# nihalsid/single-view-3d-reconstruction

Measured on AMD Instinct MI355X. Metric: query-points/sec fwd+bwd (128^3 grid, 50k pts), higher is better.
Workload: dtype f32

## Files before the change

### single-view-3d-reconstruction_amd/csrc/conv3d_bwdw_bf16.hip

```cpp
#include "common.h"
#include "f16x3.h"

namespace svr {
void colsum_launch(const float *Y, int64_t ldy, float *out, float *part, int64_t M, int64_t N, hipStream_t s);
int64_t colsum_workspace_floats(int64_t M, int64_t N);
void conv3d_bwd_weight_reduce_launch(const float *slab, float *dWp, int Ci, int Co, int cit, int cot, int parts,
                                     hipStream_t s, int param_layout, const float *dbpart, float *db, int dbparts);
}

using namespace svr;

namespace {

typedef __bf16 bf16x8 __attribute__((ext_vector_type(8)));
typedef __bf16 bf16x2 __attribute__((ext_vector_type(2)));
typedef float f32x16 __attribute__((ext_vector_type(16)));

struct ConvShape {
  int B, D, H, W, Ci, Co;
};

constexpr int BRZ = 4, BRY = 4, BRX = 8;
constexpr int HLY = BRY + 2;
constexpr int HROWS = (BRZ + 2) * (BRY + 2);
constexpr int ROWDW = 6;
constexpr int CIS = HROWS * ROWDW + 2;
constexpr int COS = BRZ * BRY * 4 + 4;
constexpr int IN_PLANE = 32 * CIS, DO_PLANE = 32 * COS;
constexpr int BUF = 2 * IN_PLANE + 2 * DO_PLANE;
constexpr int NT = 512;
constexpr int IN_ITEMS = HROWS * 5 * 8;
constexpr int DO_ITEMS = BRZ * BRY * 4 * 8;
constexpr int IN_IT = (IN_ITEMS + NT - 1) / NT;
static_assert(IN_IT == 3 && DO_ITEMS == NT, "prefetch phases below are written for 3 + 1 items per thread");
constexpr int TAPS_PER_WAVE = 7;

__device__ __forceinline__ void split2(float x0, float x1, uint32_t &hi, uint32_t &mid) {
#if defined(SVR_WG_EXP) && SVR_WG_EXP == 3
  hi = __float_as_uint(x0);
  mid = __float_as_uint(x1);
  return;
#endif
  f32x2 v = {x0, x1};
  bf16x2 h = __builtin_convertvector(v, bf16x2);
  hi = __builtin_bit_cast(uint32_t, h);
  f32x2 r = {x0 - __uint_as_float(hi << 16), x1 - __uint_as_float(hi & 0xffff0000u)};
  bf16x2 m = __builtin_convertvector(r, bf16x2);
  mid = __builtin_bit_cast(uint32_t, m);
}

__device__ __forceinline__ bf16x8 frag(uint32_t a, uint32_t b, uint32_t c, uint32_t d) {
  union { uint4 q; bf16x8 v; } f;
  f.q = make_uint4(a, b, c, d);
  return f.v;
}

template <int G, bool F16>
__device__ __forceinline__ void wgrad_rows(const uint32_t *__restrict__ ibuf, const uint32_t *__restrict__ dbuf, int l31, int r,
                                           f32x16 (&acc)[TAPS_PER_WAVE]) {
  constexpr int T0 = G * TAPS_PER_WAVE, T1 = (T0 + TAPS_PER_WAVE < 27) ? T0 + TAPS_PER_WAVE : 27;
  const int vz = r >> 2, vy = r & 3;
  const uint4 bh = *reinterpret_cast<const uint4 *>(dbuf + l31 * COS + r * 4);
  const uint4 bm = *reinterpret_cast<const uint4 *>(dbuf + DO_PLANE + l31 * COS + r * 4);
  const bf16x8 b_hi = frag(bh.x, bh.y, bh.z, bh.w), b_mid = frag(bm.x, bm.y, bm.z, bm.w);
#pragma unroll
  for (int R = T0 / 3; R <= (T1 - 1) / 3; ++R) {
    const int dzi = R / 3, dyi = R % 3;
    const uint32_t *ph = ibuf + l31 * CIS + ((vz + dzi) * HLY + vy + dyi) * ROWDW;
    const uint2 m01 = *reinterpret_cast<const uint2 *>(ph + IN_PLANE), m23 = *reinterpret_cast<const uint2 *>(ph + IN_PLANE + 2);
    const uint32_t m4 = ph[IN_PLANE + 4];
    const uint2 h01 = *reinterpret_cast<const uint2 *>(ph), h23 = *reinterpret_cast<const uint2 *>(ph + 2);
    const uint32_t h4 = ph[4];
#pragma unroll
    for (int dx = 0; dx < 3; ++dx) {
      const int tap = R * 3 + dx;
      if (tap < T0 || tap >= T1) continue;
      const int i = tap - T0;
      const bf16x8 am = dx == 0 ? frag(m01.x, m01.y, m23.x, m23.y)
                      : dx == 2 ? frag(m01.y, m23.x, m23.y, m4)
                                : frag(__builtin_amdgcn_alignbit(m01.y, m01.x, 16), __builtin_amdgcn_alignbit(m23.x, m01.y, 16),
                                       __builtin_amdgcn_alignbit(m23.y, m23.x, 16), __builtin_amdgcn_alignbit(m4, m23.y, 16));
      const bf16x8 ah = dx == 0 ? frag(h01.x, h01.y, h23.x, h23.y)
                      : dx == 2 ? frag(h01.y, h23.x, h23.y, h4)
                                : frag(__builtin_amdgcn_alignbit(h01.y, h01.x, 16), __builtin_amdgcn_alignbit(h23.x, h01.y, 16),
                                       __builtin_amdgcn_alignbit(h23.y, h23.x, 16), __builtin_amdgcn_alignbit(h4, h23.y, 16));
#if defined(SVR_WG_EXP) && SVR_WG_EXP == 1
      acc[i][0] += (float)am[0] * (float)b_hi[1] + (float)ah[2] * (float)b_mid[3] + (float)ah[7];
#else
      if constexpr (F16) {
        const f16x8 fam = __builtin_bit_cast(f16x8, am), fah = __builtin_bit_cast(f16x8, ah);
        const f16x8 fbh = __builtin_bit_cast(f16x8, b_hi), fbm = __builtin_bit_cast(f16x8, b_mid);
        acc[i] = __builtin_amdgcn_mfma_f32_32x32x16_f16(fam, scale_2m11(fbh), acc[i], 0, 0, 0);
        acc[i] = __builtin_amdgcn_mfma_f32_32x32x16_f16(scale_2m11(fah), fbm, acc[i], 0, 0, 0);
        acc[i] = __builtin_amdgcn_mfma_f32_32x32x16_f16(fah, fbh, acc[i], 0, 0, 0);
      } else {
      acc[i] = __builtin_amdgcn_mfma_f32_32x32x16_bf16(am, b_hi, acc[i], 0, 0, 0);
      acc[i] = __builtin_amdgcn_mfma_f32_32x32x16_bf16(ah, b_mid, acc[i], 0, 0, 0);
      acc[i] = __builtin_amdgcn_mfma_f32_32x32x16_bf16(ah, b_hi, acc[i], 0, 0, 0);
      }
#endif
    }
  }
}

template <bool F16>
__global__ __launch_bounds__(NT) void conv3d_bwd_weight_x3_kernel(const float *__restrict__ in,
                                                                  const float *__restrict__ dout,
                                                                  float *__restrict__ slab, ConvShape s, int nbz, int nby,
                                                                  int nbx, int co_tiles, float *__restrict__ dbpart,
                                                                  const uint32_t *__restrict__ amax_dout) {
  __shared__ uint32_t lds[2 * BUF];
  float sy = 1.f;
  if constexpr (F16) sy = amax_dout ? w_scale(amax_dout[0], false) : 1.f;
  const int t = threadIdx.x, lane = t & 63, wave = t >> 6;
  const int l31 = lane & 31, lh = lane >> 5;
  const int grp = wave & 3, half = wave >> 2;
  const int pair = blockIdx.y;
  const int ci0 = (pair / co_tiles) * 32, co0 = (pair % co_tiles) * 32;
  const int bricks = s.B * nbz * nby * nbx;

  float4 ia[2][2], da[2];
  int iok[2], dok = 0;
  const bool want_db = dbpart != nullptr && ci0 == 0;
  float4 dbs = make_float4(0.f, 0.f, 0.f, 0.f);

  auto load = [&](int brick, int ph) {
    int q = brick;
    const int bx = q % nbx; q /= nbx;
    const int by = q % nby; q /= nby;
    const int bz = q % nbz;
    const int b = q / nbz;
    const int z0 = bz * BRZ, y0 = by * BRY, x0 = bx * BRX;
    const float *inb = in + (int64_t)b * s.D * s.H * s.W * s.Ci;
#pragma unroll
    for (int j = 0; j < (ph == 0 ? 2 : 1); ++j) {
      const int idx = min(t + NT * (ph * 2 + j), IN_ITEMS - 1);
      const int hrow = idx / 40, rem = idx % 40, pr = rem >> 3, cg = rem & 7;
      const int gz = z0 + hrow / HLY - 1, gy = y0 + hrow % HLY - 1, gx = x0 + 2 * pr - 1;
      const bool rowok = gz >= 0 && gz < s.D && gy >= 0 && gy < s.H && ci0 + cg * 4 < s.Ci;
      const int cz = min(max(gz, 0), s.D - 1), cy = min(max(gy, 0), s.H - 1), cc = min(ci0 + cg * 4, s.Ci - 4);
      const uint32_t ro = __umul24(__umul24(__umul24((uint32_t)cz, (uint32_t)s.H) + (uint32_t)cy, (uint32_t)s.W), (uint32_t)s.Ci) + (uint32_t)cc;
      const char *p = reinterpret_cast<const char *>(inb);
#if defined(SVR_WG_EXP) && SVR_WG_EXP == 2
      ia[j][0] = make_float4((float)idx, 1.f, (float)brick, 3.f);
      ia[j][1] = make_float4((float)(uintptr_t)p, 1.f, 2.f, 3.f);
#else
      ia[j][0] = *reinterpret_cast<const float4 *>(p + (ro + __umul24((uint32_t)min(max(gx, 0), s.W - 1), (uint32_t)s.Ci)) * 4u);
      ia[j][1] = *reinterpret_cast<const float4 *>(p + (ro + __umul24((uint32_t)min(max(gx + 1, 0), s.W - 1), (uint32_t)s.Ci)) * 4u);
#endif
      iok[j] = (rowok && gx >= 0 && gx < s.W ? 1 : 0) | (rowok && gx + 1 >= 0 && gx + 1 < s.W ? 2 : 0);
    }
    if (ph == 1) {
      const float *dob = dout + (int64_t)b * s.D * s.H * s.W * s.Co;
      const int row = t >> 5, pr = (t & 31) >> 3, cg = t & 7;
      const int gz = z0 + (row >> 2), gy = y0 + (row & 3), gx = x0 + 2 * pr;
      const bool rowok = gz < s.D && gy < s.H && co0 + cg * 4 < s.Co;
      const int cz = min(gz, s.D - 1), cy = min(gy, s.H - 1), cc = min(co0 + cg * 4, s.Co - 4);
      const uint32_t ro = __umul24(__umul24(__umul24((uint32_t)cz, (uint32_t)s.H) + (uint32_t)cy, (uint32_t)s.W), (uint32_t)s.Co) + (uint32_t)cc;
      const char *p = reinterpret_cast<const char *>(dob);
#if defined(SVR_WG_EXP) && SVR_WG_EXP == 2
      da[0] = make_float4((float)t, 1.f, (float)brick, 3.f);
      da[1] = make_float4((float)(uintptr_t)p, 1.f, 2.f, 3.f);
#else
      da[0] = *reinterpret_cast<const float4 *>(p + (ro + __umul24((uint32_t)min(gx, s.W - 1), (uint32_t)s.Co)) * 4u);
      da[1] = *reinterpret_cast<const float4 *>(p + (ro + __umul24((uint32_t)min(gx + 1, s.W - 1), (uint32_t)s.Co)) * 4u);
#endif
      dok = (rowok && gx < s.W ? 1 : 0) | (rowok && gx + 1 < s.W ? 2 : 0);
    }
  };

  auto store = [&](uint32_t *buf, int ph) {
#pragma unroll
    for (int j = 0; j < (ph == 0 ? 2 : 1); ++j) {
      const int idx = t + NT * (ph * 2 + j);
      if (idx < IN_ITEMS) {
        const int hrow = idx / 40, rem = idx % 40, pr = rem >> 3, cg = rem & 7;
        uint32_t *d = buf + (cg * 4) * CIS + hrow * ROWDW + pr;
        const float v0[4] = {ia[j][0].x, ia[j][0].y, ia[j][0].z, ia[j][0].w};
        const float v1[4] = {ia[j][1].x, ia[j][1].y, ia[j][1].z, ia[j][1].w};
#pragma unroll
        for (int c = 0; c < 4; ++c) {
          uint32_t h, m;
          if constexpr (F16) split_x((iok[j] & 1) ? v0[c] : 0.f, (iok[j] & 2) ? v1[c] : 0.f, h, m);
          else split2((iok[j] & 1) ? v0[c] : 0.f, (iok[j] & 2) ? v1[c] : 0.f, h, m);
          d[c * CIS] = h;
          d[IN_PLANE + c * CIS] = m;
        }
      }
    }
    if (ph == 1) {
      uint32_t *dbuf = buf + 2 * IN_PLANE;
      const int row = t >> 5, pr = (t & 31) >> 3, cg = t & 7;
      uint32_t *d = dbuf + (cg * 4) * COS + row * 4 + pr;
      float v0[4] = {da[0].x, da[0].y, da[0].z, da[0].w};
      float v1[4] = {da[1].x, da[1].y, da[1].z, da[1].w};
#pragma unroll
      for (int c = 0; c < 4; ++c) {
        v0[c] = (dok & 1) ? v0[c] : 0.f;
        v1[c] = (dok & 2) ? v1[c] : 0.f;
        uint32_t h, m;
        if constexpr (F16) split_x(v0[c] * sy, v1[c] * sy, h, m);
        else split2(v0[c], v1[c], h, m);
        d[c * COS] = h;
        d[DO_PLANE + c * COS] = m;
      }
      if (want_db) {
        dbs.x += v0[0] + v1[0]; dbs.y += v0[1] + v1[1]; dbs.z += v0[2] + v1[2]; dbs.w += v0[3] + v1[3];
      }
    }
  };

  f32x16 acc[TAPS_PER_WAVE];
#pragma unroll
  for (int i = 0; i < TAPS_PER_WAVE; ++i)
#pragma unroll
    for (int r = 0; r < 16; ++r) acc[i][r] = 0.f;

  int brick = (int)blockIdx.x;
  if (brick < bricks) {
    load(brick, 0);
    store(lds, 0);
    load(brick, 1);
    store(lds, 1);
  }
  __syncthreads();
  int cur = 0;
  for (; brick < bricks; brick += (int)gridDim.x) {
    const int next = brick + (int)gridDim.x;
    const bool more = next < bricks;
    if (more) load(next, 0);
    const uint32_t *ibuf = lds + cur * BUF, *dbuf = ibuf + 2 * IN_PLANE;
#pragma unroll 1
    for (int kq = 0; kq < 4; ++kq) {
      const int r = 2 * (half * 4 + kq) + lh;
      switch (grp) {
        case 0: wgrad_rows<0, F16>(ibuf, dbuf, l31, r, acc); break;
        case 1: wgrad_rows<1, F16>(ibuf, dbuf, l31, r, acc); break;
        case 2: wgrad_rows<2, F16>(ibuf, dbuf, l31, r, acc); break;
        default: wgrad_rows<3, F16>(ibuf, dbuf, l31, r, acc); break;
      }
      if (kq == 1 && more) {
        store(lds + (cur ^ 1) * BUF, 0);
        load(next, 1);
      }
    }
    if (more) store(lds + (cur ^ 1) * BUF, 1);
    __syncthreads();
    cur ^= 1;
  }

  if (want_db) {
    float *sred = reinterpret_cast<float *>(lds);
    sred[t * 4 + 0] = dbs.x; sred[t * 4 + 1] = dbs.y; sred[t * 4 + 2] = dbs.z; sred[t * 4 + 3] = dbs.w;
    __syncthreads();
    if (t < 32) {
      const int cg = t >> 2, c = t & 3;
      float sum = 0.f;
      for (int i = 0; i < NT / 8; ++i) sum += sred[(i * 8 + cg) * 4 + c];
      if (co0 + t < s.Co) dbpart[(int64_t)blockIdx.x * s.Co + co0 + t] = sum;
    }
  }
  float inv = 1.f;
  if constexpr (F16) inv = amax_dout ? w_scale(amax_dout[0], true) : 1.f;
  const int pairs = gridDim.y;
  const int64_t part = (int64_t)blockIdx.x * 2 + half;
#pragma unroll
  for (int i = 0; i < TAPS_PER_WAVE; ++i) {
    const int tap = grp * TAPS_PER_WAVE + i;
    if (tap < 27) {
      float *o = slab + ((part * 27 + tap) * pairs + pair) * 1024;
#pragma unroll
      for (int r = 0; r < 16; ++r) o[((r & 3) + 8 * (r >> 2) + 4 * lh) * 32 + l31] = F16 ? acc[i][r] * inv : acc[i][r];
    }
  }
}

__global__ __launch_bounds__(256) void db_reduce_kernel(const float *__restrict__ dbpart, float *__restrict__ db, int Co,
                                                        int parts) {
  __shared__ double red[256];
  const int co = blockIdx.x;
  double sum = 0.0;
  for (int p = threadIdx.x; p < parts; p += 256) sum += (double)dbpart[(int64_t)p * Co + co];
  red[threadIdx.x] = sum;
  __syncthreads();
  for (int o = 128; o > 0; o >>= 1) {
    if ((int)threadIdx.x < o) red[threadIdx.x] += red[threadIdx.x + o];
    __syncthreads();
  }
  if (threadIdx.x == 0) db[co] = (float)red[0];
}

int x3_parts(int B, int D, int H, int W, int Ci, int Co) {
  int64_t bricks = (int64_t)B * cdiv(D, BRZ) * cdiv(H, BRY) * cdiv(W, BRX);
  int64_t pairs = cdiv(Ci, 32) * cdiv(Co, 32);
  int64_t parts = cdiv(256, pairs);
  if (parts > bricks) parts = bricks;
  return (int)(parts < 1 ? 1 : parts);
}

}

extern "C" int64_t svr_conv3d_k3_bwd_weight_bf16x3_workspace(int32_t B, int32_t D, int32_t H, int32_t W, int32_t Ci,
                                                             int32_t Co) {
  int64_t tiles = cdiv(Ci, 32) * cdiv(Co, 32);
  const int64_t parts = x3_parts(B, D, H, W, Ci, Co);
  return (parts * 2 * 27 * tiles * 1024 + parts * Co) * (int64_t)sizeof(float);
}

namespace {
int bwd_weight_x3(const float *in, const float *dout, float *dWp, float *db, int32_t B, int32_t D, int32_t H, int32_t W, int32_t Ci,
                  int32_t Co, void *workspace, void *stream, int param_layout, bool f16 = false, const uint32_t *amax_dout = nullptr);
}

extern "C" int svr_conv3d_k3_bwd_weight_f16x3(const float *in, const float *dout, float *dW, float *db, int32_t B, int32_t D,
                                              int32_t H, int32_t W, int32_t Ci, int32_t Co, int32_t param_layout,
                                              const uint32_t *amax_dout, void *workspace, void *stream) {
  return bwd_weight_x3(in, dout, dW, db, B, D, H, W, Ci, Co, workspace, stream, param_layout ? 1 : 0, true, amax_dout);
}

extern "C" int svr_conv3d_k3_bwd_weight_bf16x3(const float *in, const float *dout, float *dWp, float *db, int32_t B,
                                               int32_t D, int32_t H, int32_t W, int32_t Ci, int32_t Co, void *workspace,
                                               void *stream) {
  return bwd_weight_x3(in, dout, dWp, db, B, D, H, W, Ci, Co, workspace, stream, 0);
}

extern "C" int svr_conv3d_k3_bwd_weight_bf16x3_param(const float *in, const float *dout, float *dW, float *db, int32_t B,
                                                     int32_t D, int32_t H, int32_t W, int32_t Ci, int32_t Co, void *workspace,
                                                     void *stream) {
  return bwd_weight_x3(in, dout, dW, db, B, D, H, W, Ci, Co, workspace, stream, 1);
}

namespace {
int bwd_weight_x3(const float *in, const float *dout, float *dWp, float *db, int32_t B, int32_t D, int32_t H, int32_t W, int32_t Ci,
                  int32_t Co, void *workspace, void *stream, int param_layout, bool f16, const uint32_t *amax_dout) {
  SVR_CHECK(B > 0 && D > 0 && H > 0 && W > 0, SVR_E_BADSHAPE, "conv3d_bwd_weight_bf16x3: empty volume %dx%dx%dx%d", B, D, H, W);
  SVR_CHECK(in && dout && dWp && workspace, SVR_E_BADARG, "conv3d_bwd_weight_bf16x3: null pointer");
  SVR_CHECK(Ci >= 4 && Ci % 4 == 0 && Co % 4 == 0 && Co >= 4, SVR_E_UNSUPPORTED,
            "conv3d_bwd_weight_bf16x3: need Ci, Co %% 4 == 0 (Ci=%d Co=%d)", Ci, Co);
  SVR_CHECK((((uintptr_t)in | (uintptr_t)dout) & 15) == 0, SVR_E_ALIGN, "conv3d_bwd_weight_bf16x3: 16-byte alignment");
  SVR_CHECK((int64_t)D * H * W <= (1LL << 24) && (int64_t)D * H * W * (Ci > Co ? Ci : Co) < (1LL << 30) &&
                (int64_t)B * cdiv(D, BRZ) * cdiv(H, BRY) * cdiv(W, BRX) < (1LL << 31),
            SVR_E_UNSUPPORTED, "conv3d_bwd_weight_bf16x3: volume %dx%dx%dx%d too large for 32-bit offsets", B, D, H, W);
  hipStream_t s = (hipStream_t)stream;
  ConvShape sh{B, D, H, W, Ci, Co};
  const int cit = (int)cdiv(Ci, 32), cot = (int)cdiv(Co, 32);
  const int nbz = (int)cdiv(D, BRZ), nby = (int)cdiv(H, BRY), nbx = (int)cdiv(W, BRX);
  const int parts = x3_parts(B, D, H, W, Ci, Co);
  float *slab = (float *)workspace;
  float *dbpart = db ? slab + (int64_t)parts * 2 * 27 * cit * cot * 1024 : nullptr;
  if (f16)
    hipLaunchKernelGGL(conv3d_bwd_weight_x3_kernel<true>, dim3((unsigned)parts, (unsigned)(cit * cot)), dim3(NT), 0, s, in, dout,
                       slab, sh, nbz, nby, nbx, cot, dbpart, amax_dout);
  else
    hipLaunchKernelGGL(conv3d_bwd_weight_x3_kernel<false>, dim3((unsigned)parts, (unsigned)(cit * cot)), dim3(NT), 0, s, in, dout,
                       slab, sh, nbz, nby, nbx, cot, dbpart, (const uint32_t *)nullptr);
  conv3d_bwd_weight_reduce_launch(slab, dWp, Ci, Co, cit, cot, parts * 2, s, param_layout, dbpart, db, parts);
  return launch_status("conv3d_bwd_weight_bf16x3");
}
}
```

Before: 25.70 million.

## Add warp-specialized producer/consumer kernel for bf16x3 conv3d weight gradient

Adds a warp-specialized variant of the split-precision conv3d weight-gradient kernel. Four waves only load global input and dout, split them into hi/mid parts and write them into double-buffered LDS. The other four waves only run MFMA over tap groups. A paired-row mode packs two kernel rows into one 32-wide MFMA tile when Ci<=16 to avoid wasted lanes. The new path is taken when there are at least 8 bricks per part, and it halves the number of partial slabs to reduce. The aim is to overlap global loads and conversion with matrix math, at the cost of more code and half the waves doing MFMA.

```diff
diff --git a/single-view-3d-reconstruction_amd/csrc/conv3d_bwdw_bf16.hip b/single-view-3d-reconstruction_amd/csrc/conv3d_bwdw_bf16.hip
--- a/single-view-3d-reconstruction_amd/csrc/conv3d_bwdw_bf16.hip
+++ b/single-view-3d-reconstruction_amd/csrc/conv3d_bwdw_bf16.hip
@@ -275,6 +275,276 @@
   }
 }
 
+constexpr int WS_NP = NT / 2;
+
+template <int G, bool PAIR>
+struct WsFrag {
+  static constexpr int NTT = PAIR ? 15 : 27, TPW = PAIR ? 4 : TAPS_PER_WAVE;
+  static constexpr int T0 = G * TPW, T1 = (T0 + TPW < NTT) ? T0 + TPW : NTT;
+  static constexpr int RA = T0 / 3, NR = (T1 - 1) / 3 - RA + 1;
+  uint4 bh, bm;
+  uint2 m01[NR], m23[NR], h01[NR], h23[NR];
+  uint32_t m4[NR], h4[NR];
+};
+
+template <int G, bool PAIR>
+__device__ __forceinline__ void ws_fetch(const uint32_t *__restrict__ ibuf, const uint32_t *__restrict__ dbuf, int l31, int r,
+                                         WsFrag<G, PAIR> &f) {
+  using F = WsFrag<G, PAIR>;
+  const int vz = r >> 2, vy = r & 3;
+  f.bh = *reinterpret_cast<const uint4 *>(dbuf + l31 * COS + r * 4);
+  f.bm = *reinterpret_cast<const uint4 *>(dbuf + DO_PLANE + l31 * COS + r * 4);
+  const uint32_t *pl = ibuf + (PAIR ? (l31 & 15) : l31) * CIS + (vz * HLY + vy) * ROWDW;
+#pragma unroll
+  for (int k = 0; k < F::NR; ++k) {
+    const int R = F::RA + k;
+    const int ra = PAIR ? 2 * R : R, rb = PAIR ? (2 * R + 1 < 9 ? 2 * R + 1 : 8) : R;
+    const int oa = ((ra / 3) * HLY + ra % 3) * ROWDW, ob = ((rb / 3) * HLY + rb % 3) * ROWDW;
+    const uint32_t *ph = pl + (PAIR && l31 >= 16 ? ob : oa);
+    f.m01[k] = *reinterpret_cast<const uint2 *>(ph + IN_PLANE);
+    f.m23[k] = *reinterpret_cast<const uint2 *>(ph + IN_PLANE + 2);
+    f.m4[k] = ph[IN_PLANE + 4];
+    f.h01[k] = *reinterpret_cast<const uint2 *>(ph);
+    f.h23[k] = *reinterpret_cast<const uint2 *>(ph + 2);
+    f.h4[k] = ph[4];
+  }
+}
+
+template <int G, bool F16, bool PAIR>
+__device__ __forceinline__ void ws_mfma(const WsFrag<G, PAIR> &f, f32x16 (&acc)[TAPS_PER_WAVE]) {
+  using F = WsFrag<G, PAIR>;
+  const bf16x8 b_hi = frag(f.bh.x, f.bh.y, f.bh.z, f.bh.w), b_mid = frag(f.bm.x, f.bm.y, f.bm.z, f.bm.w);
+#pragma unroll
+  for (int k = 0; k < F::NR; ++k) {
+    const int R = F::RA + k;
+#pragma unroll
+    for (int dx = 0; dx < 3; ++dx) {
+      const int tt = R * 3 + dx;
+      if (tt < F::T0 || tt >= F::T1) continue;
+      const int i = tt - F::T0;
+      const uint2 m01 = f.m01[k], m23 = f.m23[k], h01 = f.h01[k], h23 = f.h23[k];
+      const uint32_t m4 = f.m4[k], h4 = f.h4[k];
+      const bf16x8 am = dx == 0 ? frag(m01.x, m01.y, m23.x, m23.y)
+                      : dx == 2 ? frag(m01.y, m23.x, m23.y, m4)
+                                : frag(__builtin_amdgcn_alignbit(m01.y, m01.x, 16), __builtin_amdgcn_alignbit(m23.x, m01.y, 16),
+                                       __builtin_amdgcn_alignbit(m23.y, m23.x, 16), __builtin_amdgcn_alignbit(m4, m23.y, 16));
+      const bf16x8 ah = dx == 0 ? frag(h01.x, h01.y, h23.x, h23.y)
+                      : dx == 2 ? frag(h01.y, h23.x, h23.y, h4)
+                                : frag(__builtin_amdgcn_alignbit(h01.y, h01.x, 16), __builtin_amdgcn_alignbit(h23.x, h01.y, 16),
+                                       __builtin_amdgcn_alignbit(h23.y, h23.x, 16), __builtin_amdgcn_alignbit(h4, h23.y, 16));
+      if constexpr (F16) {
+        const f16x8 fam = __builtin_bit_cast(f16x8, am), fah = __builtin_bit_cast(f16x8, ah);
+        const f16x8 fbh = __builtin_bit_cast(f16x8, b_hi), fbm = __builtin_bit_cast(f16x8, b_mid);
+        acc[i] = __builtin_amdgcn_mfma_f32_32x32x16_f16(fam, scale_2m11(fbh), acc[i], 0, 0, 0);
+        acc[i] = __builtin_amdgcn_mfma_f32_32x32x16_f16(scale_2m11(fah), fbm, acc[i], 0, 0, 0);
+        acc[i] = __builtin_amdgcn_mfma_f32_32x32x16_f16(fah, fbh, acc[i], 0, 0, 0);
+      } else {
+        acc[i] = __builtin_amdgcn_mfma_f32_32x32x16_bf16(am, b_hi, acc[i], 0, 0, 0);
+        acc[i] = __builtin_amdgcn_mfma_f32_32x32x16_bf16(ah, b_mid, acc[i], 0, 0, 0);
+        acc[i] = __builtin_amdgcn_mfma_f32_32x32x16_bf16(ah, b_hi, acc[i], 0, 0, 0);
+      }
+    }
+  }
+}
+
+template <int G, bool F16, bool PAIR>
+__device__ __forceinline__ void ws_consume(const uint32_t *lds, int n_it, float *__restrict__ slab, int pair,
+                                           const uint32_t *__restrict__ amax_dout) {
+  const int lane = threadIdx.x & 63, l31 = lane & 31, lh = lane >> 5;
+  f32x16 acc[TAPS_PER_WAVE];
+#pragma unroll
+  for (int i = 0; i < TAPS_PER_WAVE; ++i)
+#pragma unroll
+    for (int r = 0; r < 16; ++r) acc[i][r] = 0.f;
+  __syncthreads();
+  int cur = 0;
+  for (int it = 0; it < n_it; ++it) {
+    const uint32_t *ibuf = lds + cur * BUF, *dbuf = ibuf + 2 * IN_PLANE;
+#pragma unroll 1
+    for (int kq = 0; kq < 8; ++kq) {
+      WsFrag<G, PAIR> f;
+      ws_fetch<G, PAIR>(ibuf, dbuf, l31, 2 * kq + lh, f);
+      ws_mfma<G, F16, PAIR>(f, acc);
+    }
+    __syncthreads();
+    cur ^= 1;
+  }
+  float inv = 1.f;
+  if constexpr (F16) inv = amax_dout ? w_scale(amax_dout[0], true) : 1.f;
+  const int pairs = gridDim.y;
+  const int64_t part = blockIdx.x;
+  constexpr int NTT = PAIR ? 15 : 27, TPW = PAIR ? 4 : TAPS_PER_WAVE;
+#pragma unroll
+  for (int i = 0; i < TPW; ++i) {
+    const int tt = G * TPW + i;
+    if (tt >= NTT) continue;
+    if constexpr (PAIR) {
+      const int R = tt / 3, dx = tt % 3;
+      float *lo = slab + ((part * 27 + (2 * R) * 3 + dx) * pairs + pair) * 1024;
+      float *hi = slab + ((part * 27 + (2 * R + 1) * 3 + dx) * pairs + pair) * 1024;
+#pragma unroll
+      for (int r = 0; r < 16; ++r) {
+        const int row = (r & 3) + 8 * (r >> 2) + 4 * lh;
+        const float v = F16 ? acc[i][r] * inv : acc[i][r];
+        if (r < 8) lo[row * 32 + l31] = v;
+        else if (2 * R + 1 < 9) hi[(row - 16) * 32 + l31] = v;
+      }
+    } else {
+      float *o = slab + ((part * 27 + tt) * pairs + pair) * 1024;
+#pragma unroll
+      for (int r = 0; r < 16; ++r) o[((r & 3) + 8 * (r >> 2) + 4 * lh) * 32 + l31] = F16 ? acc[i][r] * inv : acc[i][r];
+    }
+  }
+}
+
+template <bool F16, bool PAIR>
+__global__ __launch_bounds__(NT) void conv3d_bwd_weight_ws_kernel(const float *__restrict__ in, const float *__restrict__ dout,
+                                                                  float *__restrict__ slab, ConvShape s, int nbz, int nby,
+                                                                  int nbx, int co_tiles, float *__restrict__ dbpart,
+                                                                  const uint32_t *__restrict__ amax_dout) {
+  constexpr int CG = PAIR ? 4 : 8;
+  constexpr int IN_N = HROWS * 5 * CG;
+  constexpr int IN_PT = (IN_N + WS_NP - 1) / WS_NP;
+  constexpr int DO_PT = DO_ITEMS / WS_NP;
+  static_assert(DO_ITEMS % WS_NP == 0 && WS_NP % 8 == 0, "a producer thread's dout items share one channel group");
+  __shared__ uint32_t lds[2 * BUF];
+  const int t = threadIdx.x, lane = t & 63;
+  const int wave = __builtin_amdgcn_readfirstlane(t >> 6);
+  const int pair = blockIdx.y;
+  const int ci0 = (pair / co_tiles) * 32, co0 = (pair % co_tiles) * 32;
+  const int bricks = s.B * nbz * nby * nbx;
+  const int n_it = (bricks - (int)blockIdx.x + (int)gridDim.x - 1) / (int)gridDim.x;
+  const bool want_db = dbpart != nullptr && ci0 == 0;
+  float4 dbs = make_float4(0.f, 0.f, 0.f, 0.f);
+
+  if (wave < 4) {
+    switch (wave) {
+      case 0: ws_consume<0, F16, PAIR>(lds, n_it, slab, pair, amax_dout); break;
+      case 1: ws_consume<1, F16, PAIR>(lds, n_it, slab, pair, amax_dout); break;
+      case 2: ws_consume<2, F16, PAIR>(lds, n_it, slab, pair, amax_dout); break;
+      default: ws_consume<3, F16, PAIR>(lds, n_it, slab, pair, amax_dout); break;
+    }
+  } else {
+    const int p = t - WS_NP;
+    float sy = 1.f;
+    if constexpr (F16) sy = amax_dout ? w_scale(amax_dout[0], false) : 1.f;
+    float4 ia[IN_PT][2], da[DO_PT][2];
+    int iok[IN_PT], dok[DO_PT];
+
+    auto load = [&](int brick) {
+      int q = brick;
+      const int bx = q % nbx; q /= nbx;
+      const int by = q % nby; q /= nby;
+      const int bz = q % nbz;
+      const int b = q / nbz;
+      const int z0 = bz * BRZ, y0 = by * BRY, x0 = bx * BRX;
+      const char *inb = reinterpret_cast<const char *>(in + (int64_t)b * s.D * s.H * s.W * s.Ci);
+#pragma unroll
+      for (int j = 0; j < IN_PT; ++j) {
+        const int idx = min(p + WS_NP * j, IN_N - 1);
+        const int hrow = idx / (5 * CG), rem = idx % (5 * CG), pr = rem / CG, cg = rem % CG;
+        const int gz = z0 + hrow / HLY - 1, gy = y0 + hrow % HLY - 1, gx = x0 + 2 * pr - 1;
+        const bool rowok = gz >= 0 && gz < s.D && gy >= 0 && gy < s.H && ci0 + cg * 4 < s.Ci;
+        const int cz = min(max(gz, 0), s.D - 1), cy = min(max(gy, 0), s.H - 1), cc = min(ci0 + cg * 4, s.Ci - 4);
+        const uint32_t ro = __umul24(__umul24(__umul24((uint32_t)cz, (uint32_t)s.H) + (uint32_t)cy, (uint32_t)s.W), (uint32_t)s.Ci) + (uint32_t)cc;
+        ia[j][0] = *reinterpret_cast<const float4 *>(inb + (ro + __umul24((uint32_t)min(max(gx, 0), s.W - 1), (uint32_t)s.Ci)) * 4u);
+        ia[j][1] = *reinterpret_cast<const float4 *>(inb + (ro + __umul24((uint32_t)min(max(gx + 1, 0), s.W - 1), (uint32_t)s.Ci)) * 4u);
+        iok[j] = (rowok && gx >= 0 && gx < s.W ? 1 : 0) | (rowok && gx + 1 >= 0 && gx + 1 < s.W ? 2 : 0);
+      }
+      const char *dob = reinterpret_cast<const char *>(dout + (int64_t)b * s.D * s.H * s.W * s.Co);
+#pragma unroll
+      for (int j = 0; j < DO_PT; ++j) {
+        const int idx = p + WS_NP * j;
+        const int row = idx >> 5, pr = (idx & 31) >> 3, cg = idx & 7;
+        const int gz = z0 + (row >> 2), gy = y0 + (row & 3), gx = x0 + 2 * pr;
+        const bool rowok = gz < s.D && gy < s.H && co0 + cg * 4 < s.Co;
+        const int cz = min(gz, s.D - 1), cy = min(gy, s.H - 1), cc = min(co0 + cg * 4, s.Co - 4);
+        const uint32_t ro = __umul24(__umul24(__umul24((uint32_t)cz, (uint32_t)s.H) + (uint32_t)cy, (uint32_t)s.W), (uint32_t)s.Co) + (uint32_t)cc;
+        da[j][0] = *reinterpret_cast<const float4 *>(dob + (ro + __umul24((uint32_t)min(gx, s.W - 1), (uint32_t)s.Co)) * 4u);
+        da[j][1] = *reinterpret_cast<const float4 *>(dob + (ro + __umul24((uint32_t)min(gx + 1, s.W - 1), (uint32_t)s.Co)) * 4u);
+        dok[j] = (rowok && gx < s.W ? 1 : 0) | (rowok && gx + 1 < s.W ? 2 : 0);
+      }
+    };
+
+    auto store = [&](uint32_t *buf) {
+#pragma unroll
+      for (int j = 0; j < IN_PT; ++j) {
+        const int idx = p + WS_NP * j;
+        if (IN_N % WS_NP == 0 || idx < IN_N) {
+          const int hrow = idx / (5 * CG), rem = idx % (5 * CG), pr = rem / CG, cg = rem % CG;
+          uint32_t *d = buf + (cg * 4) * CIS + hrow * ROWDW + pr;
+          const float4 a0 = ia[j][0], a1 = ia[j][1];
+          const int ok = iok[j];
+          const float v0[4] = {a0.x, a0.y, a0.z, a0.w};
+          const float v1[4] = {a1.x, a1.y, a1.z, a1.w};
+#pragma unroll
+          for (int c = 0; c < 4; ++c) {
+            uint32_t h, m;
+            if constexpr (F16) split_x((ok & 1) ? v0[c] : 0.f, (ok & 2) ? v1[c] : 0.f, h, m);
+            else split2((ok & 1) ? v0[c] : 0.f, (ok & 2) ? v1[c] : 0.f, h, m);
+            d[c * CIS] = h;
+            d[IN_PLANE + c * CIS] = m;
+          }
+        }
+      }
+      uint32_t *dbuf = buf + 2 * IN_PLANE;
+#pragma unroll
+      for (int j = 0; j < DO_PT; ++j) {
+        const int idx = p + WS_NP * j;
+        const int row = idx >> 5, pr = (idx & 31) >> 3, cg = idx & 7;
+        uint32_t *d = dbuf + (cg * 4) * COS + row * 4 + pr;
+        const float4 a0 = da[j][0], a1 = da[j][1];
+        const int ok = dok[j];
+        float v0[4] = {a0.x, a0.y, a0.z, a0.w};
+        float v1[4] = {a1.x, a1.y, a1.z, a1.w};
+#pragma unroll
+        for (int c = 0; c < 4; ++c) {
+          v0[c] = (ok & 1) ? v0[c] : 0.f;
+          v1[c] = (ok & 2) ? v1[c] : 0.f;
+          uint32_t h, m;
+          if constexpr (F16) split_x(v0[c] * sy, v1[c] * sy, h, m);
+          else split2(v0[c], v1[c], h, m);
+          d[c * COS] = h;
+          d[DO_PLANE + c * COS] = m;
+        }
+        if (want_db) {
+          dbs.x += v0[0] + v1[0]; dbs.y += v0[1] + v1[1]; dbs.z += v0[2] + v1[2]; dbs.w += v0[3] + v1[3];
+        }
+      }
+    };
+
+    const int b0 = blockIdx.x, g = gridDim.x;
+    load(b0);
+    store(lds);
+    if (n_it > 1) load(b0 + g);
+    __syncthreads();
+    int cur = 0;
+    for (int it = 0; it < n_it; ++it) {
+      if (it + 1 < n_it) {
+        store(lds + (cur ^ 1) * BUF);
+        if (it + 2 < n_it) load(b0 + (it + 2) * g);
+      }
+      __syncthreads();
+      cur ^= 1;
+    }
+  }
+
+  if (want_db) {
+    float *sred = reinterpret_cast<float *>(lds);
+    if (wave >= 4) {
+      const int p = t - WS_NP;
+      sred[p * 4 + 0] = dbs.x; sred[p * 4 + 1] = dbs.y; sred[p * 4 + 2] = dbs.z; sred[p * 4 + 3] = dbs.w;
+    }
+    __syncthreads();
+    if (t < 32) {
+      const int cg = t >> 2, c = t & 3;
+      float sum = 0.f;
+      for (int i = 0; i < WS_NP / 8; ++i) sum += sred[(i * 8 + cg) * 4 + c];
+      if (co0 + t < s.Co) dbpart[(int64_t)blockIdx.x * s.Co + co0 + t] = sum;
+    }
+  }
+}
+
 __global__ __launch_bounds__(256) void db_reduce_kernel(const float *__restrict__ dbpart, float *__restrict__ db, int Co,
                                                         int parts) {
   __shared__ double red[256];
@@ -348,6 +618,21 @@
   const int parts = x3_parts(B, D, H, W, Ci, Co);
   float *slab = (float *)workspace;
   float *dbpart = db ? slab + (int64_t)parts * 2 * 27 * cit * cot * 1024 : nullptr;
+  constexpr int WS_MIN_BRICKS = 8;
+  const int64_t nbricks = (int64_t)B * nbz * nby * nbx;
+  if (nbricks >= (int64_t)parts * WS_MIN_BRICKS) {
+    const dim3 grid((unsigned)parts, (unsigned)(cit * cot));
+    const uint32_t *am = f16 ? amax_dout : nullptr;
+    if (Ci <= 16) {
+      if (f16) hipLaunchKernelGGL((conv3d_bwd_weight_ws_kernel<true, true>), grid, dim3(NT), 0, s, in, dout, slab, sh, nbz, nby, nbx, cot, dbpart, am);
+      else hipLaunchKernelGGL((conv3d_bwd_weight_ws_kernel<false, true>), grid, dim3(NT), 0, s, in, dout, slab, sh, nbz, nby, nbx, cot, dbpart, am);
+    } else {
+      if (f16) hipLaunchKernelGGL((conv3d_bwd_weight_ws_kernel<true, false>), grid, dim3(NT), 0, s, in, dout, slab, sh, nbz, nby, nbx, cot, dbpart, am);
+      else hipLaunchKernelGGL((conv3d_bwd_weight_ws_kernel<false, false>), grid, dim3(NT), 0, s, in, dout, slab, sh, nbz, nby, nbx, cot, dbpart, am);
+    }
+    conv3d_bwd_weight_reduce_launch(slab, dWp, Ci, Co, cit, cot, parts, s, param_layout, dbpart, db, parts);
+    return launch_status("conv3d_bwd_weight_bf16x3");
+  }
   if (f16)
     hipLaunchKernelGGL(conv3d_bwd_weight_x3_kernel<true>, dim3((unsigned)parts, (unsigned)(cit * cot)), dim3(NT), 0, s, in, dout,
                        slab, sh, nbz, nby, nbx, cot, dbpart, amax_dout);
```

Result: faster. 26.09 million (median of 6 runs) (+1.5%).
